# scottberry/TmLibrary

Measured on AMD Instinct MI355X. Metric: sites/sec (2160×2560 uint16) illumstats+correct; % of HBM roofline at 1–8 GPUs, higher is better.
Workload: dtype f64 stats / f32 correct (±1 DN)

## Files before the change

### include/tmhip.h

```cpp
#ifndef TMHIP_H
#define TMHIP_H

#include <stddef.h>
#include <stdint.h>

#ifdef __cplusplus
extern "C" {
#endif

#define TMH_ABI_VERSION 7

#define TMH_OK 0
#define TMH_EINVAL (-22)
#define TMH_ENOMEM (-12)
#define TMH_EDEVICE (-5)
#define TMH_ESTATE (-71)

int tmh_abi_version(void);
const char* tmh_last_error(void);
int tmh_device_count(int* n);
int tmh_set_device(int device);
int tmh_synchronize(void* stream);

typedef struct tmh_stats tmh_stats;
// ... 1 lines not shown
#define TMH_STATS_DEFERRED_PCT 1u
#define TMH_STATS_KEEP_SITE_HIST 2u
#define TMH_STATS_SERIAL 4u

int tmh_stats_create(int height, int width, int n_quantiles, const int64_t* q_lo,
                     const int64_t* q_hi, const double* q_gamma, const double* lut_log10,
                     int batch_capacity, unsigned flags, tmh_stats** out);
void tmh_stats_destroy(tmh_stats* h);
int tmh_stats_set_stream(tmh_stats* h, void* stream);
int tmh_stats_reset(tmh_stats* h);

#define TMH_OPT_FUSED_CONFIG 1
#define TMH_OPT_WELFORD_PARTS 2
#define TMH_OPT_COPY_THREADS 4
#define TMH_OPT_HOST_STAGING 5
int tmh_stats_set_option(tmh_stats* h, int option, int value);

int tmh_stats_update(tmh_stats* h, const uint16_t* host_sites, int64_t n_sites,
                     int log_transform, int64_t* zero_counts_out);
int tmh_stats_update_device(tmh_stats* h, const uint16_t* dev_sites, int64_t n_sites,
                            int log_transform, void* stream);
int tmh_stats_zero_counts(tmh_stats* h, int64_t* host_out, int64_t n, void* stream);

int tmh_stats_update_welford_device(tmh_stats* h, const uint16_t* dev_sites, int64_t n_sites,
                                    int log_transform, void* stream);

int tmh_stats_probe_device(tmh_stats* h, const uint16_t* dev_sites, int64_t n_sites,
                           void* stream);
int tmh_stats_probe_blocks_device(tmh_stats* h, const uint16_t* const* dev_blocks, int block_shift,
                                  int64_t n_sites, void* stream);

int tmh_stats_update_welford_blocks_device(tmh_stats* h, const uint16_t* const* dev_blocks,
                                           int block_shift, int64_t n_sites, int log_transform,
                                           void* stream);

int tmh_stats_finalize(tmh_stats* h, int64_t* n, double* mean, double* std, double* pct_sum,
                       uint64_t* hist);
int tmh_stats_finalize_device(tmh_stats* h, double* dev_mean, double* dev_std, void* stream);
int tmh_stats_variance(tmh_stats* h, double* host_var);
int tmh_stats_wide_groups(tmh_stats* h, uint64_t* groups_out, int64_t* sites_out);
#define TMH_FUSED_NO_HIST 100
int tmh_stats_job_choice(tmh_stats* h, uint32_t* probe_counts, int* welford_bright,
                         int* fused_cfg);
int tmh_stats_site_histogram(tmh_stats* h, int64_t site_in_last_batch, uint32_t* host_hist);
int tmh_stats_site_order_stats(tmh_stats* h, int64_t site, uint16_t* host_vlo,
                               uint16_t* host_vhi);

int tmh_stats_get_n(tmh_stats* h, int64_t* n);
int tmh_stats_set_n(tmh_stats* h, int64_t n);
int tmh_stats_merge_stage1(tmh_stats* h, double* dev_nmean, void* stream);
int tmh_stats_merge_stage2(tmh_stats* h, const double* dev_sum_nmean, int64_t n_total,
                           double* dev_m2c, void* stream);
int tmh_stats_merge_stage3(tmh_stats* h, int64_t n_total, const double* dev_sum_m2c,
                           void* stream);
int tmh_stats_pct_accumulate(tmh_stats* h, double* dev_acc, void* stream);
// ... 194 lines not shown
```

### tmlibrary_amd/csrc/abi_internal.h

```cpp
#pragma once

#include <algorithm>
#include <vector>

#include "common.h"

#pragma GCC visibility push(hidden)

namespace tmh {

template <typename F>
inline int guard(F&& f) {
  try {
    f();
    return TMH_OK;
  } catch (const Error& e) {
    set_error(e.msg);
    return e.code;
  } catch (const std::bad_alloc&) {
    set_error("host allocation failed");
    return TMH_ENOMEM;
  } catch (...) {
    set_error("unknown error");
    return TMH_EDEVICE;
// ... 125 lines not shown
  double scale = 0.0;
  unsigned flags = 0;
  int64_t batch_cap = 0;
  hipStream_t own_stream = nullptr;
  hipStream_t stream = nullptr;
  hipStream_t side = nullptr;
  hipStream_t tail = nullptr;
  hipEvent_t ev_fork = nullptr, ev_join = nullptr;
  hipEvent_t ev_in = nullptr, ev_out = nullptr;
  static constexpr int kJoins = 8;
  hipEvent_t join_ev[kJoins]{};
  hipStream_t join_s[kJoins]{};
  int join_n = 0;
  int fused_cfg = kFusedAuto;
  int wf_parts = 0;
  HostOpts host;
  bool hist_dirty = false;
  int64_t n = 0;
  int64_t n_deferred = 0;
  int64_t last_batch = 0;
  int64_t pending = 0;
  DBuf<unsigned long long> wide;
  DBuf<unsigned int> probe;
  unsigned int* probe_host = nullptr;
  hipEvent_t ev_probe = nullptr;
  bool probed = false;
  bool probe_queued = false;
  unsigned int probe_cnt[3] = {0u, 0u, 0u};
  int64_t wide_sites = 0;
  bool pct_sum_external = false;
// ... 91 lines not shown
```

### tmlibrary_amd/csrc/abi_stats.hip

```cpp
#include <cstring>

#include "abi_internal.h"

namespace tmh {

void defer_join(tmh_stats* h, hipStream_t s) {
  int i = 0;
  while (i < h->join_n && h->join_s[i] != s) ++i;
  if (i == tmh_stats::kJoins) {
    hstream(h);
    i = 0;
  }
  hipEvent_t& e = h->join_ev[i];
  if (!e) TMH_HIP(hipEventCreateWithFlags(&e, hipEventDisableTiming));
  TMH_HIP(hipEventRecord(e, s));
  h->join_s[i] = s;
  if (i == h->join_n) ++h->join_n;
}

size_t os_words(const tmh_stats* h, int64_t n_sites) {
  return (size_t)n_sites * (size_t)os_tiles(h->Q) * kOsTile;
}

void stats_reserve_sites(tmh_stats* h, int64_t n_sites) {
// ... 79 lines not shown
    h->rn.alloc((size_t)ns);
  }
  const bool serial = (h->flags & TMH_STATS_SERIAL) != 0;
  hipStream_t hs = serial ? s : h->side;
  const int64_t chunk = 4096;
  stats_reserve_sites(h, std::min(chunk, ns));
  if (h->flags & TMH_STATS_DEFERRED_PCT) stats_grow_deferred(h, ns);
  const bool vec = (h->npx & 7) == 0 && (reinterpret_cast<uintptr_t>(d) & 15) == 0;
  if (vec && log_transform && h->wf_parts == 0 && ns >= 96) stats_probe(h, d, ns, SiteTab{}, s);
  if (!serial) {
    TMH_HIP(hipEventRecord(h->ev_fork, s));
    TMH_HIP(hipStreamWaitEvent(hs, h->ev_fork, 0));
  }
  launch_welford(d, h->npx, ns, h->n, h->rn.p, h->mean.p, h->m2.p, h->lut_log.p,
                 log_transform, h->wf_part.p, h->wf_part.n, h->wf_parts, nullptr,
                 probe_bright(h) ? 1 : 0, s);
  for (int64_t c0 = 0; c0 < ns; c0 += chunk) {
    const int64_t nc = std::min(chunk, ns - c0);
    const bool deferred = (h->flags & TMH_STATS_DEFERRED_PCT) != 0;
    uint32_t* vlh = h->vlh.p + (deferred ? (size_t)h->n_deferred * kOsTile : 0);
    const int64_t ld = deferred ? h->vlh_cap : nc;
    launch_hist_scatter(d + c0 * h->npx, h->npx, nc, h->hist_hi.p, h->qp, vlh, ld, h->pooled.p,
                        h->zeros.p, (h->flags & 2u) ? h->site_hist.p : nullptr, hs);
    if (deferred)
      h->n_deferred += nc;
    else
      launch_pct_accumulate(vlh, nc, ld, h->Q, h->gamma.p, h->acc.p, hs);
    h->vlh_ld = ld;
    h->last_batch = nc;
  }
  if (!serial) {
// ... 4 lines not shown
}

static void stats_welford_dev(tmh_stats* h, const uint16_t* dev_sites, int64_t n_sites,
                              int log_transform, void* stream, const SiteTab& tab) {
  hipStream_t s = hpick(h, stream);
  cross_begin(h, s);
  if ((size_t)n_sites > h->rn.n) {
    TMH_HIP(hipStreamSynchronize(s));
    h->rn.alloc((size_t)n_sites);
  }
  const bool vec = tab.in || ((h->npx & 7) == 0 && (reinterpret_cast<uintptr_t>(dev_sites) & 15) == 0);
  if (vec && (h->fused_cfg == kFusedAuto || (log_transform && h->wf_parts == 0)))
    stats_probe(h, dev_sites, n_sites, tab, s);
  launch_welford(dev_sites, h->npx, n_sites, h->n, h->rn.p, h->mean.p, h->m2.p, h->lut_log.p,
                 log_transform, h->wf_part.p, h->wf_part.n, h->wf_parts, h->wide.p,
                 probe_bright(h) ? 1 : 0, s, -1, tab);
  if ((h->npx & 7) == 0) h->wide_sites += n_sites;
  h->n += n_sites;
  h->pending += n_sites;
  cross_end(h, s);
}

SiteTab blocked_tab(const uint16_t* const* dev_in_blocks, uint16_t* const* dev_out_blocks,
                    int block_shift, int64_t npx) {
  TMH_CHECK(dev_in_blocks, TMH_EINVAL, "block table is NULL");
  TMH_CHECK(block_shift >= 2 && block_shift <= 24, TMH_EINVAL, "block_shift must be 2..24");
  TMH_CHECK((npx & 7) == 0, TMH_EINVAL,
            "blocked site layouts need height * width divisible by 8 (16-byte pixel groups)");
  SiteTab t;
  t.in = dev_in_blocks;
  t.out = dev_out_blocks;
// ... 114 lines not shown
}

int tmh_stats_set_option(tmh_stats* h, int option, int value) {
  return guard([&] {
    TMH_CHECK(h, TMH_EINVAL, "handle is NULL");
    switch (option) {
      case TMH_OPT_FUSED_CONFIG:
        TMH_CHECK((value >= kFusedAuto && value < kFusedConfigs) || value == kFusedNoHist,
                  TMH_EINVAL, "fused configuration out of range");
        h->fused_cfg = value;
        break;
      case TMH_OPT_WELFORD_PARTS:
        TMH_CHECK(value >= 0 && value <= 4, TMH_EINVAL, "Welford parts must be 0..4");
        h->wf_parts = value;
        break;
      default:
        if (!h->host.set(option, value)) throw Error{TMH_EINVAL, "unknown option"};
    }
  });
}

int tmh_stats_reset(tmh_stats* h) {
  return guard([&] {
    TMH_CHECK(h, TMH_EINVAL, "handle is NULL");
    if (h->hist_dirty) {
      TMH_HIP(hipDeviceSynchronize());
      if (h->hist_full.n)
        TMH_HIP(hipMemsetAsync(h->hist_full.p, 0, h->hist_full.n * 4, hstream(h)));
      if (h->hist_rmask.n)
        TMH_HIP(hipMemsetAsync(h->hist_rmask.p, 0, h->hist_rmask.n * 8, hstream(h)));
// ... 193 lines not shown
    }
  });
}

int tmh_stats_wide_groups(tmh_stats* h, uint64_t* groups_out, int64_t* sites_out) {
  return guard([&] {
    TMH_CHECK(h && groups_out, TMH_EINVAL, "bad arguments");
    unsigned long long w = 0;
    TMH_HIP(hipMemcpyAsync(&w, h->wide.p, 8, hipMemcpyDeviceToHost, hstream(h)));
    TMH_HIP(hipStreamSynchronize(hstream(h)));
    *groups_out = w;
    if (sites_out) *sites_out = h->wide_sites;
  });
}

int tmh_stats_get_hist_device(tmh_stats* h, uint64_t* dev_hist, void* stream) {
  return guard([&] {
    TMH_CHECK(h && dev_hist, TMH_EINVAL, "bad arguments");
    const hipStream_t s = hpick(h, stream);
    cross_begin(h, s);
    TMH_HIP(hipMemcpyAsync(dev_hist, h->pooled.p, (size_t)kBins * 8, hipMemcpyDeviceToDevice, s));
    cross_end(h, s);
  });
}

int tmh_stats_set_hist_device(tmh_stats* h, const uint64_t* dev_hist, void* stream) {
  return guard([&] {
    TMH_CHECK(h && dev_hist, TMH_EINVAL, "bad arguments");
    const hipStream_t s = hpick(h, stream);
    cross_begin(h, s);
// ... 139 lines not shown
```

### tmlibrary_amd/csrc/common.h

```cpp
#pragma once

#include <hip/hip_runtime.h>

#include <cstdint>
#include <cstdio>
#include <string>

#include "../../include/tmhip.h"

namespace tmh {

void set_error(const std::string& msg);

struct Error {
  int code;
  std::string msg;
};

#define TMH_HIP(expr)                                                                    \
  do {                                                                                   \
    hipError_t _e = (expr);                                                              \
    if (_e != hipSuccess)                                                                \
      throw ::tmh::Error{TMH_EDEVICE, std::string(#expr) + ": " + hipGetErrorString(_e)}; \
  } while (0)
// ... 93 lines not shown
  int shift = 0;
};

struct RareList {
  uint16_t* v = nullptr;
  unsigned int* cnt = nullptr;
  unsigned int cap = 0;
};
constexpr int kRareLo = 16384;

__device__ __forceinline__ int64_t site_block(const SiteTab& t, int64_t s) { return s >> t.shift; }
__device__ __forceinline__ int64_t site_in_block(const SiteTab& t, int64_t s) {
  return s & ((1ll << t.shift) - 1);
}

void launch_welford(const uint16_t* sites, int64_t npx, int64_t n_sites, int64_t n0, double* rn,
                    double* mean, double* m2, const double* lut, int log_transform,
                    double* part, size_t part_cap, int forced_parts,
                    unsigned long long* wide, int bright, hipStream_t s, int shape = -1,
                    const SiteTab& tab = SiteTab{});
void launch_site_probe(const uint16_t* sites, int64_t npx, int64_t n_sites, unsigned int* out,
                       hipStream_t s, const SiteTab& tab = SiteTab{});
void launch_hist_scatter(const uint16_t* sites, int64_t npx, int64_t n_sites, uint32_t* hist_hi,
                         const QPos& p, uint32_t* vlh, int64_t vlh_ld, unsigned long long* pooled,
                         int64_t* zero_counts, uint32_t* site_hist, hipStream_t s);
constexpr int kPooledParts = 16;
void launch_hist_site_u16(const uint16_t* sites, int64_t npx, int64_t n_sites, uint32_t* slab,
                          const QPos& p, uint32_t* vlh, int64_t vlh_ld,
                          unsigned long long* pooled, unsigned long long* pooled_parts,
                          int64_t* zero_counts, uint32_t* site_hist, hipStream_t s,
// ... 215 lines not shown
```

### tmlibrary_amd/csrc/stats_kernels.hip

```cpp
#include <algorithm>

#include "common.h"
#include "hist_tail.h"

namespace tmh {


constexpr double kInvLn10 = 0.43429448190325182765;
constexpr double kLog10_16 = 1.2041199826559247809;
constexpr int kWfInvScalar = 2;
template <int INV>
__device__ __forceinline__ double recip16(uint32_t a, const double* sinv) {
  if (INV == 1) return sinv[a];
  const double d = (double)(a << 4);
  const double r0 = (double)__builtin_amdgcn_rcpf((float)(a << 4));
  return fma(r0, fma(-d, r0, 1.0), r0);
}
template <int INV>
__device__ __forceinline__ double log10_big(uint32_t u, const double* slut, const double* sinv) {
  const uint32_t a = u >> 4;
  if (INV == 2) {
    constexpr float c1 = (float)kInvLn10, c2 = (float)(-0.5 * kInvLn10),
                    c3 = (float)(kInvLn10 / 3.0);
    const float t = (float)(u & 15u) * __builtin_amdgcn_rcpf((float)(a << 4));
// ... 34 lines not shown

template <bool LOG>
__device__ __forceinline__ double xform(uint32_t u, const double* slut) {
  if (!LOG) return (double)u;
  double x = slut[u & (uint32_t)(kWfLut - 1)];
  if (u >= (uint32_t)kWfLut) x = log10_big<kWfInvScalar>(u, slut, nullptr);
  return x;
}

__device__ __forceinline__ void welford1(double x, double rn, double& mu, double& m2) {
  const double d = x - mu;
  mu = fma(d, rn, mu);
  m2 = fma(d, x - mu, m2);
}

constexpr int kWfThreads = 256;
constexpr int kWfInv = 2;
constexpr int kWfScalarThreads = 256;
constexpr int kWfGroup = 2;
constexpr int kWfMaxParts = 4;

__global__ void k_rn_table(double* __restrict__ rn, int64_t n0, int64_t n) {
  const int64_t i = (int64_t)blockIdx.x * 256 + threadIdx.x;
  if (i < n) rn[i] = 1.0 / (double)(n0 + i + 1);
}

__device__ __forceinline__ void lut_offsets(uint32_t m, uint32_t three, uint32_t& lo,
                                            uint32_t& hi) {
  asm("v_lshlrev_b32_sdwa %0, %1, %2 dst_sel:DWORD dst_unused:UNUSED_PAD src0_sel:DWORD "
      "src1_sel:WORD_0"
      : "=v"(lo)
// ... 4 lines not shown
      : "v"(three), "v"(m));
}
typedef unsigned short u16x2_t __attribute__((ext_vector_type(2)));
__device__ __forceinline__ uint32_t pk_min_u16(uint32_t w, uint32_t c2) {
  return __builtin_bit_cast(uint32_t, __builtin_elementwise_min(__builtin_bit_cast(u16x2_t, w),
                                                                __builtin_bit_cast(u16x2_t, c2)));
}
__device__ __forceinline__ uint32_t pk_max_u16(uint32_t a, uint32_t b) {
  return __builtin_bit_cast(uint32_t, __builtin_elementwise_max(__builtin_bit_cast(u16x2_t, a),
                                                                __builtin_bit_cast(u16x2_t, b)));
}
__device__ __forceinline__ double lds_at(const double* base, uint32_t byte_off) {
  return *reinterpret_cast<const double*>(reinterpret_cast<const char*>(base) + byte_off);
}

template <bool LOG, int INV, int LUTN = kWfLut>
__device__ __forceinline__ void xform8(const uint4 v, const double* slut, const double* sinv,
                                       double (&x)[8], uint32_t& wc, uint32_t& xc) {
  const uint32_t u[8] = {v.x & 0xFFFFu, v.x >> 16, v.y & 0xFFFFu, v.y >> 16,
                         v.z & 0xFFFFu, v.z >> 16, v.w & 0xFFFFu, v.w >> 16};
  const uint32_t any = v.x | v.y | v.z | v.w;
  const bool wide = (any & 0xF000F000u) != 0;
  constexpr bool kPow2 = (LUTN & (LUTN - 1)) == 0;
  constexpr uint32_t kIdx = LUTN - 1;
  if (LOG) {
    const uint32_t wd[4] = {v.x, v.y, v.z, v.w};
    const uint32_t three = 3u;
    constexpr uint32_t kIdx2 = kIdx * 0x00010001u;
#pragma unroll
    for (int p = 0; p < 4; ++p) {
      uint32_t lo, hi;
      lut_offsets(kPow2 ? wd[p] & kIdx2 : pk_min_u16(wd[p], kIdx2), three, lo, hi);
      x[2 * p] = lds_at(slut, lo);
      x[2 * p + 1] = lds_at(slut, hi);
    }
  }
  if (LOG && LUTN == kWfLutBright) {
    wc += wide ? 1u : 0u;
    xc += (any & 0xC000C000u) ? 1u : 0u;
    const uint32_t mx = pk_max_u16(pk_max_u16(v.x, v.y), pk_max_u16(v.z, v.w));
    if ((mx & 0xFFFFu) > kIdx || (mx >> 16) > kIdx) {
#pragma unroll
      for (int k = 0; k < 8; ++k)
        if (u[k] > kIdx) x[k] = log10_big<INV>(u[k], slut, sinv);
    }
  } else if (LOG) {
    if (wide) {
      ++wc;
      xc += (any & 0xC000C000u) ? 1u : 0u;
#pragma unroll
      for (int k = 0; k < 8; ++k)
        if (u[k] > kIdx) x[k] = log10_big<INV>(u[k], slut, sinv);
    }
  } else {
    wc += wide ? 1u : 0u;
    xc += (any & 0xC000C000u) ? 1u : 0u;
#pragma unroll
    for (int k = 0; k < 8; ++k) x[k] = (double)u[k];
  }
}

struct WfMerge {
  double inv_nl;
  double w_new;
  double w_cross;
  int first;
};

template <bool NTL>
__device__ __forceinline__ uint4 ld_site(const uint4* p) {
  if (!NTL) return *p;
  typedef unsigned int u32x4w_t __attribute__((ext_vector_type(4)));
  const u32x4w_t v = __builtin_nontemporal_load(reinterpret_cast<const u32x4w_t*>(p));
  return make_uint4(v.x, v.y, v.z, v.w);
}

typedef unsigned int u32x4g_t __attribute__((ext_vector_type(4)));
typedef __attribute__((address_space(1))) const u32x4g_t gsite_t;
__device__ __forceinline__ gsite_t* to_global(const void* p) { return (gsite_t*)p; }
template <bool NTL>
__device__ __forceinline__ uint4 ld_site(gsite_t* p) {
  const u32x4g_t v = NTL ? __builtin_nontemporal_load(p) : *p;
  return make_uint4(v.x, v.y, v.z, v.w);
}

template <bool LOG, bool NTL, int NT, int INV, bool BLK = false, int G = kWfGroup,
          int LUTN = kWfLut>
__global__ __launch_bounds__(NT) void k_welford_vec8(
    const uint16_t* __restrict__ sites, int64_t npx, int64_t n_total, int64_t per,
    const WfMerge mg, double* __restrict__ mean, double* __restrict__ m2,
    const double* __restrict__ lut, double* __restrict__ part,
    unsigned long long* __restrict__ wide, const SiteTab tab) {
  const int parts = (int)gridDim.y;
  __shared__ double slut[LUTN], sinv[INV == 1 ? kWfLut : 1];
  __shared__ uint32_t wide_sh[2];
  if (LOG) fill_wf_tables<INV, LUTN>(lut, slut, sinv, NT);
  if (threadIdx.x < 2) wide_sh[threadIdx.x] = 0u;
  __syncthreads();
  const int64_t ngroups = npx >> 3;
  const int64_t g = (int64_t)blockIdx.x * NT + threadIdx.x;
  if (g >= ngroups) return;

  const int64_t s_begin = (int64_t)blockIdx.y * per;
  const int64_t n_sites = n_total - s_begin < per ? n_total - s_begin : per;
  const uint4* src = reinterpret_cast<const uint4*>(sites) + s_begin * ngroups + g;
  const int64_t last = n_sites - 1;
  int64_t bt = 0;
  const uint4* bbase = nullptr;
  if (BLK)
    bbase = reinterpret_cast<const uint4*>(tab.in[s_begin >> tab.shift]) +
            (s_begin & ((1ll << tab.shift) - 1)) * ngroups;
  auto site = [&](int64_t t) -> gsite_t* {
    if (!BLK) return to_global(src + t * ngroups);
    if (t != bt) {
      bt = t;
      const int64_t gs = s_begin + t;
      if (gs & ((1ll << tab.shift) - 1))
        bbase += ngroups;
      else
        bbase = reinterpret_cast<const uint4*>(tab.in[gs >> tab.shift]);
    }
    return to_global(bbase + g);
  };
  uint4 cur[G], nxt[G];
#pragma unroll
  for (int k = 0; k < G; ++k) cur[k] = ld_site<NTL>(site(k < last ? k : last));
  double K[8], s1[8], s2[8];
  uint32_t wc = 0, xc = 0;
  xform8<LOG, INV, LUTN>(cur[0], slut, sinv, K, wc, xc);
  wc = xc = 0;
#pragma unroll
  for (int k = 0; k < 8; ++k) s1[k] = s2[k] = 0.0;
  const int ns = (int)n_sites;
  auto fold = [&](const uint4 (&v)[G], int s) {
#pragma unroll
    for (int k = 0; k < G; ++k) {
      if (s + k < ns) {
        double x[8];
        xform8<LOG, INV, LUTN>(v[k], slut, sinv, x, wc, xc);
#pragma unroll
        for (int j = 0; j < 8; ++j) {
          const double d = x[j] - K[j];
          s1[j] += d;
          s2[j] = fma(d, d, s2[j]);
        }
      }
    }
  };
  auto issue = [&](uint4 (&v)[G], int s) {
#pragma unroll
    for (int k = 0; k < G; ++k) {
      const int t = s + k;
      v[k] = ld_site<NTL>(site(t < (int)last ? t : (int)last));
    }
  };
  for (int s = 0; s < ns; s += 2 * G) {
    issue(nxt, s + G);
    fold(cur, s);
    if (s + G >= ns) break;
    issue(cur, s + 2 * G);
    fold(nxt, s + G);
  }

  if (wide) {
    if (wc) atomicAdd(&wide_sh[0], wc);
    if (xc) atomicAdd(&wide_sh[1], xc);
    __syncthreads();
    if (threadIdx.x == 0 && wide_sh[0]) atomicAdd(wide, (unsigned long long)wide_sh[0]);
    if (threadIdx.x == 0 && wide_sh[1]) atomicAdd(wide + 1, (unsigned long long)wide_sh[1]);
  }

  if (parts > 1) {
    const double inv = 1.0 / (double)n_sites;
    double2* pm = reinterpret_cast<double2*>(part + (2 * blockIdx.y) * npx) + g * 4;
    double2* pq = reinterpret_cast<double2*>(part + (2 * blockIdx.y + 1) * npx) + g * 4;
#pragma unroll
    for (int k = 0; k < 4; ++k) {
      double a[2], b[2];
#pragma unroll
      for (int i = 0; i < 2; ++i) {
        const int j = 2 * k + i;
        a[i] = K[j] + s1[j] * inv;
        b[i] = fmax(s2[j] - s1[j] * (s1[j] * inv), 0.0);
      }
      pm[k] = make_double2(a[0], a[1]);
      pq[k] = make_double2(b[0], b[1]);
    }
    return;
  }
  double2* om = reinterpret_cast<double2*>(mean) + g * 4;
  double2* oq = reinterpret_cast<double2*>(m2) + g * 4;
  double mu[8], q[8];
  if (!mg.first) {
#pragma unroll
    for (int k = 0; k < 4; ++k) {
      const double2 a = om[k], b = oq[k];
      mu[2 * k] = a.x; mu[2 * k + 1] = a.y;
      q[2 * k] = b.x; q[2 * k + 1] = b.y;
    }
  }
#pragma unroll
  for (int j = 0; j < 8; ++j) {
    const double ml = K[j] + s1[j] * mg.inv_nl;
    const double m2l = fmax(s2[j] - s1[j] * (s1[j] * mg.inv_nl), 0.0);
    if (mg.first) {
      mu[j] = ml;
      q[j] = m2l;
    } else {
      const double d = ml - mu[j];
      mu[j] = fma(d, mg.w_new, mu[j]);
      q[j] = q[j] + m2l + d * d * mg.w_cross;
    }
  }
#pragma unroll
  for (int k = 0; k < 4; ++k) {
    om[k] = make_double2(mu[2 * k], mu[2 * k + 1]);
    oq[k] = make_double2(q[2 * k], q[2 * k + 1]);
  }
}

struct WfParts {
  double cnt[kWfMaxParts];
  int n;
};

__global__ void k_wf_merge_parts(const double* __restrict__ part, int64_t npx, const WfParts pc,
                                 double n0, double* __restrict__ mean, double* __restrict__ m2) {
  const int64_t i = (int64_t)blockIdx.x * 256 + threadIdx.x;
  if (i >= npx) return;
  double na = pc.cnt[0], ma = part[i], qa = part[npx + i];
// ... 27 lines not shown
  double mu = mean[p], q = m2[p];
  for (int64_t s = 0; s < n_sites; ++s)
    welford1(xform<LOG>(sites[s * npx + p], slut), rn[s], mu, q);
  mean[p] = mu;
  m2[p] = q;
}

static int welford_parts(int64_t n_sites, int64_t npx, size_t part_cap, int forced) {
  auto fits = [&](int f) {
    return f >= 1 && f <= kWfMaxParts && (f == 1 || ((size_t)2 * f * npx <= part_cap &&
                                                    n_sites >= (int64_t)f * 32));
  };
  return forced && fits(forced) ? forced : 1;
}

template <int NT, int INV, int G = kWfGroup, int LUTN = kWfLut>
static void launch_welford_vec8(const uint16_t* sites, int64_t npx, int64_t n_sites, int64_t per,
                                int f, const WfMerge& mg, double* mean, double* m2,
                                const double* lut, int log_transform, double* part,
                                unsigned long long* wide, hipStream_t s,
                                const SiteTab& tab = SiteTab{}) {
  const dim3 grid((unsigned)cdiv(npx >> 3, NT), (unsigned)f);
#define TMH_WF(L_, B_)                                                                           \
  hipLaunchKernelGGL((k_welford_vec8<L_, true, NT, INV, B_, G, LUTN>), grid, dim3(NT), 0, s,     \
                     sites, npx, n_sites, per, mg, mean, m2, lut, part, wide, tab)
  if (tab.in) {
    if (log_transform)
      TMH_WF(true, true);
    else
      TMH_WF(false, true);
  } else {
    if (log_transform)
      TMH_WF(true, false);
    else
      TMH_WF(false, false);
  }
#undef TMH_WF
}

constexpr int kProbeGroups = 16384;
// ... 46 lines not shown
                    double* mean, double* m2, const double* lut, int log_transform,
                    double* part, size_t part_cap, int forced_parts,
                    unsigned long long* wide, int bright, hipStream_t s, int shape,
                    const SiteTab& tab) {
  if (n_sites <= 0) return;
  const bool vec = tab.in || ((npx & 7) == 0 && (reinterpret_cast<uintptr_t>(sites) & 15) == 0);
  if (vec) {
    int f = part ? welford_parts(n_sites, npx, part_cap, forced_parts) : 1;
    const bool bpass = bright > 0 && part && !forced_parts && log_transform && shape < 0 &&
                       welford_parts(n_sites, npx, part_cap, kWfBrightParts) == kWfBrightParts;
    if (bpass) f = kWfBrightParts;
    const int64_t per = cdiv(n_sites, f);
    const double nl = (double)n_sites, n = (double)(n0 + n_sites);
    const WfMerge mg{1.0 / nl, nl / n, (double)n0 * nl / n, n0 == 0};
    ProfScope prof("welford", s);
    switch (shape) {
      case 0: launch_welford_vec8<256, 0>(sites, npx, n_sites, per, f, mg, mean, m2, lut, log_transform, part, wide, s); break;
      case 1: launch_welford_vec8<256, 1>(sites, npx, n_sites, per, f, mg, mean, m2, lut, log_transform, part, wide, s); break;
      case 2: launch_welford_vec8<512, 0>(sites, npx, n_sites, per, f, mg, mean, m2, lut, log_transform, part, wide, s); break;
      case 3: launch_welford_vec8<512, 1>(sites, npx, n_sites, per, f, mg, mean, m2, lut, log_transform, part, wide, s); break;
      case 4: launch_welford_vec8<256, 2>(sites, npx, n_sites, per, f, mg, mean, m2, lut, log_transform, part, wide, s); break;
      case 5: launch_welford_vec8<512, 2>(sites, npx, n_sites, per, f, mg, mean, m2, lut, log_transform, part, wide, s); break;
      case 6: launch_welford_vec8<256, 2, 3>(sites, npx, n_sites, per, f, mg, mean, m2, lut, log_transform, part, wide, s); break;
      case 7: launch_welford_vec8<256, 2, 4>(sites, npx, n_sites, per, f, mg, mean, m2, lut, log_transform, part, wide, s); break;
      case 8: launch_welford_vec8<512, 2, 4>(sites, npx, n_sites, per, f, mg, mean, m2, lut, log_transform, part, wide, s); break;
      default:
        if (bpass)
          launch_welford_vec8<kWfThreadsBright, kWfInv, kWfGroup, kWfLutBright>(
              sites, npx, n_sites, per, f, mg, mean, m2, lut, log_transform, part, wide, s, tab);
        else
          launch_welford_vec8<kWfThreads, kWfInv>(sites, npx, n_sites, per, f, mg, mean, m2, lut,
                                                  log_transform, part, wide, s, tab);
        break;
    }
    if (f > 1) {
      WfParts pc{};
      pc.n = f;
      for (int p = 0; p < f; ++p)
        pc.cnt[p] = (double)std::min<int64_t>(per, n_sites - (int64_t)p * per);
      hipLaunchKernelGGL(k_wf_merge_parts, dim3((unsigned)cdiv(npx, 256)), dim3(256), 0, s, part,
                         npx, pc, (double)n0, mean, m2);
    }
  } else {
    const dim3 grid((unsigned)cdiv(npx, kWfScalarThreads));
    hipLaunchKernelGGL(k_rn_table, dim3((unsigned)cdiv(n_sites, 256)), dim3(256), 0, s, rn, n0,
                       n_sites);
    if (log_transform)
// ... 469 lines not shown
```

### tmlibrary_amd/hip/__init__.py

```python
from __future__ import annotations

import ctypes as C
import os
import threading

import numpy as np

_HERE = os.path.dirname(os.path.abspath(__file__))
LIB_PATH = os.environ.get("TMH_LIB", os.path.join(_HERE, "libtmhip.so"))

TMH_OK = 0
TMH_EINVAL = -22
TMH_ENOMEM = -12
TMH_EDEVICE = -5
TMH_ESTATE = -71
TMH_STATS_DEFERRED_PCT = 1
TMH_STATS_KEEP_SITE_HIST = 2
TMH_STATS_SERIAL = 4
TMH_OPT_FUSED_CONFIG = 1
TMH_OPT_WELFORD_PARTS = 2
TMH_OPT_COPY_THREADS = 4
TMH_OPT_HOST_STAGING = 5
TMH_OPT_FUSED_CUS = 8
TMH_OPT_FUSED_BANDS = 9
TMH_FUSED_NO_HIST = 100
TMH_SYNTH_STANDARD = 0
TMH_SYNTH_BRIGHT = 1
TMH_SYNTH_UNIFORM = 2
ABI_VERSION = 7

_P = C.c_void_p
_I64 = C.c_int64
_I = C.c_int
_D = C.c_double

SIGNATURES = {
    "tmh_abi_version": (_I, []),
    "tmh_last_error": (C.c_char_p, []),
    "tmh_device_count": (_I, [C.POINTER(_I)]),
    "tmh_set_device": (_I, [_I]),
    "tmh_synchronize": (_I, [_P]),
    "tmh_stats_create": (_I, [_I, _I, _I, _P, _P, _P, _P, _I, C.c_uint, C.POINTER(_P)]),
    "tmh_stats_destroy": (None, [_P]),
    "tmh_stats_set_stream": (_I, [_P, _P]),
    "tmh_stats_reset": (_I, [_P]),
    "tmh_stats_set_option": (_I, [_P, _I, _I]),
    "tmh_stats_variance": (_I, [_P, _P]),
    "tmh_stats_wide_groups": (_I, [_P, _P, _P]),
    "tmh_stats_job_choice": (_I, [_P, _P, _P, _P]),
    "tmh_stats_get_hist_device": (_I, [_P, _P, _P]),
    "tmh_stats_set_hist_device": (_I, [_P, _P, _P]),
    "tmh_stats_update": (_I, [_P, _P, _I64, _I, _P]),
    "tmh_stats_update_device": (_I, [_P, _P, _I64, _I, _P]),
    "tmh_stats_zero_counts": (_I, [_P, _P, _I64, _P]),
    "tmh_stats_update_welford_device": (_I, [_P, _P, _I64, _I, _P]),
    "tmh_stats_probe_device": (_I, [_P, _P, _I64, _P]),
    "tmh_stats_probe_blocks_device": (_I, [_P, _P, _I, _I64, _P]),
    "tmh_corrector_update_multi_device": (_I, [_P, _I, _P, _P, _P]),
    "tmh_job_planes_multi_device": (_I, [_P, _P, _I, _P, _P, _P, _P, _D, _P]),
    "tmh_stats_update_welford_blocks_device": (_I, [_P, _P, _I, _I64, _I, _P]),
    "tmh_stats_finalize": (_I, [_P, _P, _P, _P, _P, _P]),
    "tmh_stats_finalize_device": (_I, [_P, _P, _P, _P]),
    "tmh_stats_site_histogram": (_I, [_P, _I64, _P]),
# ... 171 lines not shown
```

Before: 170,600.

## Add 4-pixel-per-thread Welford kernel variants and make shape 4 the default

Generalises the Welford kernel so each thread can handle 4 pixels instead of 8, using either 8-byte loads or paired 16-byte loads exchanged with permlane32 swaps, and adds occupancy hints via launch bounds. The wide-value counting moves from shared-memory atomics to a wave reduction, with a ballot used to avoid double counting between paired threads. The non-bright default now uses shape 4 (256 threads, INV=2), and a runtime option selects among sixteen shapes. The intent is to lower register pressure and raise memory-level parallelism; the cost is more shuffle and ballot work and a changed default configuration.

```diff
diff --git a/include/tmhip.h b/include/tmhip.h
--- a/include/tmhip.h
+++ b/include/tmhip.h
@@ -39,6 +39,7 @@
 #define TMH_OPT_WELFORD_PARTS 2
 #define TMH_OPT_COPY_THREADS 4
 #define TMH_OPT_HOST_STAGING 5
+#define TMH_OPT_WELFORD_SHAPE 10
 int tmh_stats_set_option(tmh_stats* h, int option, int value);
 
 int tmh_stats_update(tmh_stats* h, const uint16_t* host_sites, int64_t n_sites,
@@ -64,6 +65,7 @@
 int tmh_stats_finalize_device(tmh_stats* h, double* dev_mean, double* dev_std, void* stream);
 int tmh_stats_variance(tmh_stats* h, double* host_var);
 int tmh_stats_wide_groups(tmh_stats* h, uint64_t* groups_out, int64_t* sites_out);
+int tmh_stats_very_wide_groups(tmh_stats* h, uint64_t* groups_out);
 #define TMH_FUSED_NO_HIST 100
 int tmh_stats_job_choice(tmh_stats* h, uint32_t* probe_counts, int* welford_bright,
                          int* fused_cfg);
diff --git a/tmlibrary_amd/csrc/abi_internal.h b/tmlibrary_amd/csrc/abi_internal.h
--- a/tmlibrary_amd/csrc/abi_internal.h
+++ b/tmlibrary_amd/csrc/abi_internal.h
@@ -163,6 +163,7 @@
   int join_n = 0;
   int fused_cfg = kFusedAuto;
   int wf_parts = 0;
+  int wf_shape = -1;
   HostOpts host;
   bool hist_dirty = false;
   int64_t n = 0;
diff --git a/tmlibrary_amd/csrc/abi_stats.hip b/tmlibrary_amd/csrc/abi_stats.hip
--- a/tmlibrary_amd/csrc/abi_stats.hip
+++ b/tmlibrary_amd/csrc/abi_stats.hip
@@ -117,7 +117,7 @@
   }
   launch_welford(d, h->npx, ns, h->n, h->rn.p, h->mean.p, h->m2.p, h->lut_log.p,
                  log_transform, h->wf_part.p, h->wf_part.n, h->wf_parts, nullptr,
-                 probe_bright(h) ? 1 : 0, s);
+                 probe_bright(h) ? 1 : 0, s, h->wf_shape);
   for (int64_t c0 = 0; c0 < ns; c0 += chunk) {
     const int64_t nc = std::min(chunk, ns - c0);
     const bool deferred = (h->flags & TMH_STATS_DEFERRED_PCT) != 0;
@@ -152,7 +152,7 @@
     stats_probe(h, dev_sites, n_sites, tab, s);
   launch_welford(dev_sites, h->npx, n_sites, h->n, h->rn.p, h->mean.p, h->m2.p, h->lut_log.p,
                  log_transform, h->wf_part.p, h->wf_part.n, h->wf_parts, h->wide.p,
-                 probe_bright(h) ? 1 : 0, s, -1, tab);
+                 probe_bright(h) ? 1 : 0, s, h->wf_shape, tab);
   if ((h->npx & 7) == 0) h->wide_sites += n_sites;
   h->n += n_sites;
   h->pending += n_sites;
@@ -297,6 +297,10 @@
         TMH_CHECK(value >= 0 && value <= 4, TMH_EINVAL, "Welford parts must be 0..4");
         h->wf_parts = value;
         break;
+      case TMH_OPT_WELFORD_SHAPE:
+        TMH_CHECK(value >= -1 && value < kWfShapes, TMH_EINVAL, "Welford shape out of range");
+        h->wf_shape = value;
+        break;
       default:
         if (!h->host.set(option, value)) throw Error{TMH_EINVAL, "unknown option"};
     }
@@ -520,6 +524,16 @@
   });
 }
 
+int tmh_stats_very_wide_groups(tmh_stats* h, uint64_t* groups_out) {
+  return guard([&] {
+    TMH_CHECK(h && groups_out, TMH_EINVAL, "bad arguments");
+    unsigned long long w = 0;
+    TMH_HIP(hipMemcpyAsync(&w, h->wide.p + 1, 8, hipMemcpyDeviceToHost, hstream(h)));
+    TMH_HIP(hipStreamSynchronize(hstream(h)));
+    *groups_out = w;
+  });
+}
+
 int tmh_stats_get_hist_device(tmh_stats* h, uint64_t* dev_hist, void* stream) {
   return guard([&] {
     TMH_CHECK(h && dev_hist, TMH_EINVAL, "bad arguments");
diff --git a/tmlibrary_amd/csrc/common.h b/tmlibrary_amd/csrc/common.h
--- a/tmlibrary_amd/csrc/common.h
+++ b/tmlibrary_amd/csrc/common.h
@@ -131,6 +131,7 @@
   return s & ((1ll << t.shift) - 1);
 }
 
+constexpr int kWfShapes = 16;
 void launch_welford(const uint16_t* sites, int64_t npx, int64_t n_sites, int64_t n0, double* rn,
                     double* mean, double* m2, const double* lut, int log_transform,
                     double* part, size_t part_cap, int forced_parts,
diff --git a/tmlibrary_amd/csrc/stats_kernels.hip b/tmlibrary_amd/csrc/stats_kernels.hip
--- a/tmlibrary_amd/csrc/stats_kernels.hip
+++ b/tmlibrary_amd/csrc/stats_kernels.hip
@@ -72,7 +72,7 @@
   m2 = fma(d, x - mu, m2);
 }
 
-constexpr int kWfThreads = 256;
+constexpr int kWfShape = 4;
 constexpr int kWfInv = 2;
 constexpr int kWfScalarThreads = 256;
 constexpr int kWfGroup = 2;
@@ -107,21 +107,40 @@
   return *reinterpret_cast<const double*>(reinterpret_cast<const char*>(base) + byte_off);
 }
 
-template <bool LOG, int INV, int LUTN = kWfLut>
-__device__ __forceinline__ void xform8(const uint4 v, const double* slut, const double* sinv,
-                                       double (&x)[8], uint32_t& wc, uint32_t& xc) {
-  const uint32_t u[8] = {v.x & 0xFFFFu, v.x >> 16, v.y & 0xFFFFu, v.y >> 16,
-                         v.z & 0xFFFFu, v.z >> 16, v.w & 0xFFFFu, v.w >> 16};
-  const uint32_t any = v.x | v.y | v.z | v.w;
+template <bool LOG, int INV, int LUTN = kWfLut, int PX = 8>
+__device__ __forceinline__ void xform8(const uint32_t (&wd)[PX / 2], const double* slut,
+                                       const double* sinv, double (&x)[PX], uint32_t& wc,
+                                       uint32_t& xc, uint32_t mate = 0u) {
+  static_assert(PX == 8 || (PX == 4 && LUTN == kWfLut), "4-pixel threads: the standard table");
+  uint32_t u[PX];
+  uint32_t any = 0u;
+#pragma unroll
+  for (int p = 0; p < PX / 2; ++p) {
+    u[2 * p] = wd[p] & 0xFFFFu;
+    u[2 * p + 1] = wd[p] >> 16;
+    any |= wd[p];
+  }
   const bool wide = (any & 0xF000F000u) != 0;
+  const bool xwide = (any & 0xC000C000u) != 0;
   constexpr bool kPow2 = (LUTN & (LUTN - 1)) == 0;
   constexpr uint32_t kIdx = LUTN - 1;
+  auto count = [&]() {
+    if (PX == 8) {
+      wc += wide ? 1u : 0u;
+      xc += xwide ? 1u : 0u;
+    } else {
+      const uint32_t lane = __lane_id();
+      const bool low = lane < mate;
+      const bool mw = (__ballot(wide) >> mate) & 1ull, mx = (__ballot(xwide) >> mate) & 1ull;
+      wc += (wide && (low || !mw)) ? 1u : 0u;
+      xc += (xwide && (low || !mx)) ? 1u : 0u;
+    }
+  };
   if (LOG) {
-    const uint32_t wd[4] = {v.x, v.y, v.z, v.w};
     const uint32_t three = 3u;
     constexpr uint32_t kIdx2 = kIdx * 0x00010001u;
 #pragma unroll
-    for (int p = 0; p < 4; ++p) {
+    for (int p = 0; p < PX / 2; ++p) {
       uint32_t lo, hi;
       lut_offsets(kPow2 ? wd[p] & kIdx2 : pk_min_u16(wd[p], kIdx2), three, lo, hi);
       x[2 * p] = lds_at(slut, lo);
@@ -129,28 +148,33 @@
     }
   }
   if (LOG && LUTN == kWfLutBright) {
-    wc += wide ? 1u : 0u;
-    xc += (any & 0xC000C000u) ? 1u : 0u;
-    const uint32_t mx = pk_max_u16(pk_max_u16(v.x, v.y), pk_max_u16(v.z, v.w));
+    count();
+    uint32_t mx = wd[0];
+#pragma unroll
+    for (int p = 1; p < PX / 2; ++p) mx = pk_max_u16(mx, wd[p]);
     if ((mx & 0xFFFFu) > kIdx || (mx >> 16) > kIdx) {
 #pragma unroll
-      for (int k = 0; k < 8; ++k)
+      for (int k = 0; k < PX; ++k)
         if (u[k] > kIdx) x[k] = log10_big<INV>(u[k], slut, sinv);
     }
   } else if (LOG) {
     if (wide) {
-      ++wc;
-      xc += (any & 0xC000C000u) ? 1u : 0u;
-#pragma unroll
-      for (int k = 0; k < 8; ++k)
+      count();
+#pragma unroll
+      for (int k = 0; k < PX; ++k)
         if (u[k] > kIdx) x[k] = log10_big<INV>(u[k], slut, sinv);
     }
   } else {
-    wc += wide ? 1u : 0u;
-    xc += (any & 0xC000C000u) ? 1u : 0u;
-#pragma unroll
-    for (int k = 0; k < 8; ++k) x[k] = (double)u[k];
-  }
+    count();
+#pragma unroll
+    for (int k = 0; k < PX; ++k) x[k] = (double)u[k];
+  }
+}
+template <bool LOG, int INV, int LUTN = kWfLut>
+__device__ __forceinline__ void xform8(const uint4 v, const double* slut, const double* sinv,
+                                       double (&x)[8], uint32_t& wc, uint32_t& xc) {
+  const uint32_t wd[4] = {v.x, v.y, v.z, v.w};
+  xform8<LOG, INV, LUTN, 8>(wd, slut, sinv, x, wc, xc);
 }
 
 struct WfMerge {
@@ -176,75 +200,158 @@
   const u32x4g_t v = NTL ? __builtin_nontemporal_load(p) : *p;
   return make_uint4(v.x, v.y, v.z, v.w);
 }
+typedef unsigned int u32x2g_t __attribute__((ext_vector_type(2)));
+typedef __attribute__((address_space(1))) const u32x2g_t gsite2_t;
+template <bool NTL>
+__device__ __forceinline__ uint2 ld_site8(const void* p) {
+  const u32x2g_t v = NTL ? __builtin_nontemporal_load((gsite2_t*)p) : *(gsite2_t*)p;
+  return make_uint2(v.x, v.y);
+}
+
+__device__ __forceinline__ uint32_t wave_sum(uint32_t v) {
+#pragma unroll
+  for (int off = 32; off > 0; off >>= 1) v += (uint32_t)__shfl_xor((int)v, off, 64);
+  return v;
+}
 
 template <bool LOG, bool NTL, int NT, int INV, bool BLK = false, int G = kWfGroup,
-          int LUTN = kWfLut>
-__global__ __launch_bounds__(NT) void k_welford_vec8(
+          int LUTN = kWfLut, int PX = 8, int LD = 0, int WPS = 0>
+__global__ __launch_bounds__(NT, WPS ? WPS : 1) void k_welford_vec8(
     const uint16_t* __restrict__ sites, int64_t npx, int64_t n_total, int64_t per,
     const WfMerge mg, double* __restrict__ mean, double* __restrict__ m2,
     const double* __restrict__ lut, double* __restrict__ part,
     unsigned long long* __restrict__ wide, const SiteTab tab) {
+  static_assert(PX == 8 || PX == 4, "pixels per thread");
+  static_assert(PX == 8 ? LD == 0 : (LD == 0 || (LD == 1 && G % 2 == 0)), "site load form");
+  constexpr int W = PX / 2;
   const int parts = (int)gridDim.y;
-  __shared__ double slut[LUTN], sinv[INV == 1 ? kWfLut : 1];
-  __shared__ uint32_t wide_sh[2];
-  if (LOG) fill_wf_tables<INV, LUTN>(lut, slut, sinv, NT);
-  if (threadIdx.x < 2) wide_sh[threadIdx.x] = 0u;
+  __shared__ double slut[LUTN + (INV == 1 ? kWfLut : 0)];
+  const double* sinv = slut + LUTN;
+  if (LOG) fill_wf_tables<INV, LUTN>(lut, slut, slut + LUTN, NT);
   __syncthreads();
   const int64_t ngroups = npx >> 3;
-  const int64_t g = (int64_t)blockIdx.x * NT + threadIdx.x;
-  if (g >= ngroups) return;
+  const int64_t tid = (int64_t)blockIdx.x * NT + threadIdx.x;
+  const uint32_t lane = threadIdx.x & 63u;
+  int64_t g = tid;
+  uint32_t hh = 0u, mate = 0u;
+  if (PX == 4 && LD == 0) {
+    g = tid >> 1;
+    hh = lane & 1u;
+    mate = lane ^ 1u;
+  } else if (PX == 4) {
+    g = (tid >> 6) * 32 + (lane & 31u);
+    hh = lane >> 5;
+    mate = lane ^ 32u;
+  }
+  const bool live = g < ngroups;
+  if (!live) g = ngroups - 1;
+  const int64_t px0 = g * 8 + hh * 4;
 
   const int64_t s_begin = (int64_t)blockIdx.y * per;
   const int64_t n_sites = n_total - s_begin < per ? n_total - s_begin : per;
-  const uint4* src = reinterpret_cast<const uint4*>(sites) + s_begin * ngroups + g;
+  const int64_t sbytes = npx * 2;
+  const int64_t loff = (PX == 4 && LD == 0) ? px0 * 2 : g * 16;
+  const char* src = reinterpret_cast<const char*>(sites) + s_begin * sbytes + loff;
   const int64_t last = n_sites - 1;
   int64_t bt = 0;
-  const uint4* bbase = nullptr;
+  const char* bbase = nullptr;
   if (BLK)
-    bbase = reinterpret_cast<const uint4*>(tab.in[s_begin >> tab.shift]) +
-            (s_begin & ((1ll << tab.shift) - 1)) * ngroups;
-  auto site = [&](int64_t t) -> gsite_t* {
-    if (!BLK) return to_global(src + t * ngroups);
+    bbase = reinterpret_cast<const char*>(tab.in[s_begin >> tab.shift]) +
+            (s_begin & ((1ll << tab.shift) - 1)) * sbytes;
+  auto site = [&](int64_t t) -> const char* {
+    if (!BLK) return src + t * sbytes;
     if (t != bt) {
       bt = t;
       const int64_t gs = s_begin + t;
       if (gs & ((1ll << tab.shift) - 1))
-        bbase += ngroups;
+        bbase += sbytes;
       else
-        bbase = reinterpret_cast<const uint4*>(tab.in[gs >> tab.shift]);
-    }
-    return to_global(bbase + g);
+        bbase = reinterpret_cast<const char*>(tab.in[gs >> tab.shift]);
+    }
+    return bbase + loff;
   };
-  uint4 cur[G], nxt[G];
-#pragma unroll
-  for (int k = 0; k < G; ++k) cur[k] = ld_site<NTL>(site(k < last ? k : last));
-  double K[8], s1[8], s2[8];
+  struct Stage {
+    uint32_t w[G * W];
+  };
+  auto issue = [&](Stage& v, int s) {
+    if (PX == 4 && LD == 1) {
+#pragma unroll
+      for (int j = 0; j < G / 2; ++j) {
+        const int t0 = s + 2 * j, t1 = t0 + 1;
+        const char* p0 = site(t0 < (int)last ? t0 : (int)last);
+        const char* p1 = site(t1 < (int)last ? t1 : (int)last);
+        const uint4 q = ld_site<NTL>(to_global(hh ? p1 : p0));
+        v.w[4 * j] = q.x; v.w[4 * j + 1] = q.y; v.w[4 * j + 2] = q.z; v.w[4 * j + 3] = q.w;
+      }
+    } else {
+#pragma unroll
+      for (int k = 0; k < G; ++k) {
+        const int t = s + k;
+        const char* p = site(t < (int)last ? t : (int)last);
+        if (PX == 8) {
+          const uint4 q = ld_site<NTL>(to_global(p));
+          v.w[4 * k] = q.x; v.w[4 * k + 1] = q.y; v.w[4 * k + 2] = q.z; v.w[4 * k + 3] = q.w;
+        } else {
+          const uint2 q = ld_site8<NTL>(p);
+          v.w[2 * k] = q.x; v.w[2 * k + 1] = q.y;
+        }
+      }
+    }
+  };
+  auto ready = [&](Stage& v) {
+    if (PX == 4 && LD == 1) {
+#pragma unroll
+      for (int j = 0; j < G / 2; ++j) {
+#pragma unroll
+        for (int i = 0; i < 2; ++i) {
+          const auto r = __builtin_amdgcn_permlane32_swap(v.w[4 * j + i], v.w[4 * j + 2 + i],
+                                                          false, false);
+          v.w[4 * j + i] = r[0];
+          v.w[4 * j + 2 + i] = r[1];
+        }
+      }
+    }
+  };
+  auto words = [&](const Stage& v, int k, uint32_t (&wd)[W]) {
+#pragma unroll
+    for (int i = 0; i < W; ++i) wd[i] = v.w[k * W + i];
+  };
+  Stage cur, nxt;
+  double K[PX], s1[PX], s2[PX];
   uint32_t wc = 0, xc = 0;
-  xform8<LOG, INV, LUTN>(cur[0], slut, sinv, K, wc, xc);
+  {
+    uint32_t kw[W];
+    if (PX == 4 && LD == 1) {
+      const uint2 q = ld_site8<NTL>(site(0) + hh * 8);
+      kw[0] = q.x;
+      kw[1] = q.y;
+      issue(cur, 0);
+    } else {
+      issue(cur, 0);
+      words(cur, 0, kw);
+    }
+    xform8<LOG, INV, LUTN, PX>(kw, slut, sinv, K, wc, xc, mate);
+  }
   wc = xc = 0;
 #pragma unroll
-  for (int k = 0; k < 8; ++k) s1[k] = s2[k] = 0.0;
+  for (int k = 0; k < PX; ++k) s1[k] = s2[k] = 0.0;
   const int ns = (int)n_sites;
-  auto fold = [&](const uint4 (&v)[G], int s) {
+  auto fold = [&](Stage& v, int s) {
+    ready(v);
 #pragma unroll
     for (int k = 0; k < G; ++k) {
       if (s + k < ns) {
-        double x[8];
-        xform8<LOG, INV, LUTN>(v[k], slut, sinv, x, wc, xc);
-#pragma unroll
-        for (int j = 0; j < 8; ++j) {
+        double x[PX];
+        uint32_t wd[W];
+        words(v, k, wd);
+        xform8<LOG, INV, LUTN, PX>(wd, slut, sinv, x, wc, xc, mate);
+#pragma unroll
+        for (int j = 0; j < PX; ++j) {
           const double d = x[j] - K[j];
           s1[j] += d;
           s2[j] = fma(d, d, s2[j]);
         }
       }
-    }
-  };
-  auto issue = [&](uint4 (&v)[G], int s) {
-#pragma unroll
-    for (int k = 0; k < G; ++k) {
-      const int t = s + k;
-      v[k] = ld_site<NTL>(site(t < (int)last ? t : (int)last));
     }
   };
   for (int s = 0; s < ns; s += 2 * G) {
@@ -256,19 +363,32 @@
   }
 
   if (wide) {
-    if (wc) atomicAdd(&wide_sh[0], wc);
-    if (xc) atomicAdd(&wide_sh[1], xc);
+    const uint32_t wsum = wave_sum(live ? wc : 0u), xsum = wave_sum(live ? xc : 0u);
+    uint32_t* sums = reinterpret_cast<uint32_t*>(slut);
     __syncthreads();
-    if (threadIdx.x == 0 && wide_sh[0]) atomicAdd(wide, (unsigned long long)wide_sh[0]);
-    if (threadIdx.x == 0 && wide_sh[1]) atomicAdd(wide + 1, (unsigned long long)wide_sh[1]);
-  }
+    if (lane == 0) {
+      sums[2 * (threadIdx.x >> 6)] = wsum;
+      sums[2 * (threadIdx.x >> 6) + 1] = xsum;
+    }
+    __syncthreads();
+    if (threadIdx.x == 0) {
+      uint32_t w = 0u, x = 0u;
+      for (int i = 0; i < NT / 64; ++i) {
+        w += sums[2 * i];
+        x += sums[2 * i + 1];
+      }
+      if (w) atomicAdd(wide, (unsigned long long)w);
+      if (x) atomicAdd(wide + 1, (unsigned long long)x);
+    }
+  }
+  if (!live) return;
 
   if (parts > 1) {
     const double inv = 1.0 / (double)n_sites;
-    double2* pm = reinterpret_cast<double2*>(part + (2 * blockIdx.y) * npx) + g * 4;
-    double2* pq = reinterpret_cast<double2*>(part + (2 * blockIdx.y + 1) * npx) + g * 4;
-#pragma unroll
-    for (int k = 0; k < 4; ++k) {
+    double2* pm = reinterpret_cast<double2*>(part + (2 * blockIdx.y) * npx + px0);
+    double2* pq = reinterpret_cast<double2*>(part + (2 * blockIdx.y + 1) * npx + px0);
+#pragma unroll
+    for (int k = 0; k < W; ++k) {
       double a[2], b[2];
 #pragma unroll
       for (int i = 0; i < 2; ++i) {
@@ -281,19 +401,19 @@
     }
     return;
   }
-  double2* om = reinterpret_cast<double2*>(mean) + g * 4;
-  double2* oq = reinterpret_cast<double2*>(m2) + g * 4;
-  double mu[8], q[8];
+  double2* om = reinterpret_cast<double2*>(mean + px0);
+  double2* oq = reinterpret_cast<double2*>(m2 + px0);
+  double mu[PX], q[PX];
   if (!mg.first) {
 #pragma unroll
-    for (int k = 0; k < 4; ++k) {
+    for (int k = 0; k < W; ++k) {
       const double2 a = om[k], b = oq[k];
       mu[2 * k] = a.x; mu[2 * k + 1] = a.y;
       q[2 * k] = b.x; q[2 * k + 1] = b.y;
     }
   }
 #pragma unroll
-  for (int j = 0; j < 8; ++j) {
+  for (int j = 0; j < PX; ++j) {
     const double ml = K[j] + s1[j] * mg.inv_nl;
     const double m2l = fmax(s2[j] - s1[j] * (s1[j] * mg.inv_nl), 0.0);
     if (mg.first) {
@@ -306,7 +426,7 @@
     }
   }
 #pragma unroll
-  for (int k = 0; k < 4; ++k) {
+  for (int k = 0; k < W; ++k) {
     om[k] = make_double2(mu[2 * k], mu[2 * k + 1]);
     oq[k] = make_double2(q[2 * k], q[2 * k + 1]);
   }
@@ -364,16 +484,18 @@
   return forced && fits(forced) ? forced : 1;
 }
 
-template <int NT, int INV, int G = kWfGroup, int LUTN = kWfLut>
+template <int NT, int INV, int G = kWfGroup, int LUTN = kWfLut, int PX = 8, int LD = 0, int WPS = 0>
 static void launch_welford_vec8(const uint16_t* sites, int64_t npx, int64_t n_sites, int64_t per,
                                 int f, const WfMerge& mg, double* mean, double* m2,
                                 const double* lut, int log_transform, double* part,
                                 unsigned long long* wide, hipStream_t s,
                                 const SiteTab& tab = SiteTab{}) {
-  const dim3 grid((unsigned)cdiv(npx >> 3, NT), (unsigned)f);
+  const int64_t ng = npx >> 3;
+  const int64_t nthr = PX == 8 ? ng : LD == 0 ? 2 * ng : cdiv(ng, (int64_t)32) * 64;
+  const dim3 grid((unsigned)cdiv(nthr, (int64_t)NT), (unsigned)f);
 #define TMH_WF(L_, B_)                                                                           \
-  hipLaunchKernelGGL((k_welford_vec8<L_, true, NT, INV, B_, G, LUTN>), grid, dim3(NT), 0, s,     \
-                     sites, npx, n_sites, per, mg, mean, m2, lut, part, wide, tab)
+  hipLaunchKernelGGL((k_welford_vec8<L_, true, NT, INV, B_, G, LUTN, PX, LD, WPS>), grid,        \
+                     dim3(NT), 0, s, sites, npx, n_sites, per, mg, mean, m2, lut, part, wide, tab)
   if (tab.in) {
     if (log_transform)
       TMH_WF(true, true);
@@ -450,23 +572,26 @@
     const double nl = (double)n_sites, n = (double)(n0 + n_sites);
     const WfMerge mg{1.0 / nl, nl / n, (double)n0 * nl / n, n0 == 0};
     ProfScope prof("welford", s);
-    switch (shape) {
-      case 0: launch_welford_vec8<256, 0>(sites, npx, n_sites, per, f, mg, mean, m2, lut, log_transform, part, wide, s); break;
-      case 1: launch_welford_vec8<256, 1>(sites, npx, n_sites, per, f, mg, mean, m2, lut, log_transform, part, wide, s); break;
-      case 2: launch_welford_vec8<512, 0>(sites, npx, n_sites, per, f, mg, mean, m2, lut, log_transform, part, wide, s); break;
-      case 3: launch_welford_vec8<512, 1>(sites, npx, n_sites, per, f, mg, mean, m2, lut, log_transform, part, wide, s); break;
-      case 4: launch_welford_vec8<256, 2>(sites, npx, n_sites, per, f, mg, mean, m2, lut, log_transform, part, wide, s); break;
-      case 5: launch_welford_vec8<512, 2>(sites, npx, n_sites, per, f, mg, mean, m2, lut, log_transform, part, wide, s); break;
-      case 6: launch_welford_vec8<256, 2, 3>(sites, npx, n_sites, per, f, mg, mean, m2, lut, log_transform, part, wide, s); break;
-      case 7: launch_welford_vec8<256, 2, 4>(sites, npx, n_sites, per, f, mg, mean, m2, lut, log_transform, part, wide, s); break;
-      case 8: launch_welford_vec8<512, 2, 4>(sites, npx, n_sites, per, f, mg, mean, m2, lut, log_transform, part, wide, s); break;
+    switch (shape >= 0 ? shape : bpass ? -1 : kWfShape) {
+      case 0: launch_welford_vec8<256, 0>(sites, npx, n_sites, per, f, mg, mean, m2, lut, log_transform, part, wide, s, tab); break;
+      case 1: launch_welford_vec8<256, 1>(sites, npx, n_sites, per, f, mg, mean, m2, lut, log_transform, part, wide, s, tab); break;
+      case 2: launch_welford_vec8<512, 0>(sites, npx, n_sites, per, f, mg, mean, m2, lut, log_transform, part, wide, s, tab); break;
+      case 3: launch_welford_vec8<512, 1>(sites, npx, n_sites, per, f, mg, mean, m2, lut, log_transform, part, wide, s, tab); break;
+      case 4: launch_welford_vec8<256, 2>(sites, npx, n_sites, per, f, mg, mean, m2, lut, log_transform, part, wide, s, tab); break;
+      case 5: launch_welford_vec8<512, 2>(sites, npx, n_sites, per, f, mg, mean, m2, lut, log_transform, part, wide, s, tab); break;
+      case 6: launch_welford_vec8<256, 2, 3>(sites, npx, n_sites, per, f, mg, mean, m2, lut, log_transform, part, wide, s, tab); break;
+      case 7: launch_welford_vec8<256, 2, 4>(sites, npx, n_sites, per, f, mg, mean, m2, lut, log_transform, part, wide, s, tab); break;
+      case 8: launch_welford_vec8<512, 2, 4>(sites, npx, n_sites, per, f, mg, mean, m2, lut, log_transform, part, wide, s, tab); break;
+      case 9: launch_welford_vec8<256, 2, 4, kWfLut, 4, 0, 5>(sites, npx, n_sites, per, f, mg, mean, m2, lut, log_transform, part, wide, s, tab); break;
+      case 10: launch_welford_vec8<512, 2, 4, kWfLut, 4, 0, 6>(sites, npx, n_sites, per, f, mg, mean, m2, lut, log_transform, part, wide, s, tab); break;
+      case 11: launch_welford_vec8<512, 2, 2, kWfLut, 4, 0, 8>(sites, npx, n_sites, per, f, mg, mean, m2, lut, log_transform, part, wide, s, tab); break;
+      case 12: launch_welford_vec8<256, 2, 4, kWfLut, 4, 1, 5>(sites, npx, n_sites, per, f, mg, mean, m2, lut, log_transform, part, wide, s, tab); break;
+      case 13: launch_welford_vec8<512, 2, 4, kWfLut, 4, 1, 6>(sites, npx, n_sites, per, f, mg, mean, m2, lut, log_transform, part, wide, s, tab); break;
+      case 14: launch_welford_vec8<512, 2, 2, kWfLut, 4, 1, 8>(sites, npx, n_sites, per, f, mg, mean, m2, lut, log_transform, part, wide, s, tab); break;
+      case 15: launch_welford_vec8<256, 2, 2, kWfLut, 8, 0, 5>(sites, npx, n_sites, per, f, mg, mean, m2, lut, log_transform, part, wide, s, tab); break;
       default:
-        if (bpass)
-          launch_welford_vec8<kWfThreadsBright, kWfInv, kWfGroup, kWfLutBright>(
-              sites, npx, n_sites, per, f, mg, mean, m2, lut, log_transform, part, wide, s, tab);
-        else
-          launch_welford_vec8<kWfThreads, kWfInv>(sites, npx, n_sites, per, f, mg, mean, m2, lut,
-                                                  log_transform, part, wide, s, tab);
+        launch_welford_vec8<kWfThreadsBright, kWfInv, kWfGroup, kWfLutBright>(
+            sites, npx, n_sites, per, f, mg, mean, m2, lut, log_transform, part, wide, s, tab);
         break;
     }
     if (f > 1) {
diff --git a/tmlibrary_amd/hip/__init__.py b/tmlibrary_amd/hip/__init__.py
--- a/tmlibrary_amd/hip/__init__.py
+++ b/tmlibrary_amd/hip/__init__.py
@@ -23,6 +23,7 @@
 TMH_OPT_HOST_STAGING = 5
 TMH_OPT_FUSED_CUS = 8
 TMH_OPT_FUSED_BANDS = 9
+TMH_OPT_WELFORD_SHAPE = 10
 TMH_FUSED_NO_HIST = 100
 TMH_SYNTH_STANDARD = 0
 TMH_SYNTH_BRIGHT = 1
@@ -47,6 +48,7 @@
     "tmh_stats_set_option": (_I, [_P, _I, _I]),
     "tmh_stats_variance": (_I, [_P, _P]),
     "tmh_stats_wide_groups": (_I, [_P, _P, _P]),
+    "tmh_stats_very_wide_groups": (_I, [_P, _P]),
     "tmh_stats_job_choice": (_I, [_P, _P, _P, _P]),
     "tmh_stats_get_hist_device": (_I, [_P, _P, _P]),
     "tmh_stats_set_hist_device": (_I, [_P, _P, _P]),
```

Result: no change. 170,800, median of 6 (+0.1%).
